# gillet-thomas/NeuroViT

Hardware: AMD Instinct MI355X
Metric: fMRI volumes/sec (fwd+bwd) ViT3D 128^3 p16 d768 L12 [timed step = fwd+bwd+AdamW update] (higher is better)
Workload: dtype bf16; 1 GPU; ViT3D-base 128^3 patch 16, train step (fwd+bwd+AdamW), batch 4/GPU, dropout 0; global_batch=4, parallelism=dp1, grad_buckets=7, grad_allreduce=none (1 GPU)

## Files before the change

### neurovit_amd/_cabi.py

```python
from __future__ import annotations

import ctypes
import os
import re
from typing import Dict, List, Tuple

_HERE = os.path.dirname(os.path.abspath(__file__))
HEADER = os.path.join(os.path.dirname(_HERE), "include", "neurovit_hip.h")
LIB_PATH = os.environ.get("NEUROVIT_HIP_LIB") or os.path.join(_HERE, "lib", "libneurovit_hip.so")

_SCALARS = {"int": ctypes.c_int, "long": ctypes.c_long, "float": ctypes.c_float, "double": ctypes.c_double}


class VitConfig(ctypes.Structure):
    _fields_ = [("image_size", ctypes.c_int), ("image_patch_size", ctypes.c_int), ("frames", ctypes.c_int),
                ("frame_patch_size", ctypes.c_int), ("channels", ctypes.c_int), ("num_classes", ctypes.c_int),
                ("dim", ctypes.c_int), ("depth", ctypes.c_int), ("heads", ctypes.c_int), ("dim_head", ctypes.c_int),
                ("mlp_dim", ctypes.c_int), ("ln_eps", ctypes.c_float), ("pool_mean", ctypes.c_int),
                ("image_width", ctypes.c_int), ("patch_width", ctypes.c_int),
                ("no_proj_dropout", ctypes.c_int)]


class VitInput(ctypes.Structure):
    _fields_ = [("vol_sigma", ctypes.c_void_p), ("time_points", ctypes.c_int), ("rows_form", ctypes.c_int), ("attn_export", ctypes.c_void_p)]
# ... 47 lines not shown
ABI_VERSION = 8


def parse_header(path: str = HEADER) -> Dict[str, Tuple[object, List[object]]]:
    src = open(path).read()
    src = re.sub(r"/\*.*?\*/", " ", src, flags=re.S)
    protos = {}
    for m in re.finditer(r"\b(int|long|const char\s*\*)\s+(nv_\w+)\s*\(([^;{]*?)\)\s*;", src, flags=re.S):
        ret, name, args = m.group(1), m.group(2), " ".join(m.group(3).split())
        restype = ctypes.c_char_p if "char" in ret else _SCALARS[ret]
        argtypes = []
        if args and args != "void":
            for a in args.split(","):
                a = a.strip()
                if "*" in a:
                    argtypes.append(ctypes.c_char_p if re.match(r"const char\s*\*", a) else ctypes.c_void_p)
                elif a.startswith("unsigned long"):
                    argtypes.append(ctypes.c_ulong)
                else:
                    argtypes.append(_SCALARS[a.split()[0]])
        protos[name] = (restype, argtypes)
    return protos


class _Lib:
    def __init__(self):
        self._dll = None
        self.protos = parse_header()

    def load(self):
        if self._dll is None:
            if not os.path.exists(LIB_PATH):
                raise RuntimeError(
                    f"neurovit_amd: {LIB_PATH} not found - build it with `python -c 'import __graft_entry__ as g; g.build()'` "
                    "(or `make -C neurovit_amd/csrc`). There is no CPU / PyTorch fallback for this path.")
            dll = ctypes.CDLL(LIB_PATH)
            for name, (restype, argtypes) in self.protos.items():
                fn = getattr(dll, name)
                fn.restype, fn.argtypes = restype, argtypes
            got = dll.nv_abi_version()
            if got != ABI_VERSION:
                raise RuntimeError(f"neurovit_amd: {LIB_PATH} has ABI revision {got}, this binding expects {ABI_VERSION} - rebuild the library "
                                   "(make -C neurovit_amd/csrc); see INTEGRATION.md 'ABI revisions'")
            if os.environ.get("NEUROVIT_ATTN_MODE"):
                dll.nv_attn_set_mode(int(os.environ["NEUROVIT_ATTN_MODE"]))
            if os.environ.get("NEUROVIT_ADAMW_WGS"):
                dll.nv_gemm_set_tile(12, int(os.environ["NEUROVIT_ADAMW_WGS"]))
            if os.environ.get("NEUROVIT_HEAD_STEP"):
                dll.nv_vit_set_head_step(int(os.environ["NEUROVIT_HEAD_STEP"]))
            if os.environ.get("NEUROVIT_WGRAD_WGS"):
                dll.nv_gemm_set_tile(14, int(os.environ["NEUROVIT_WGRAD_WGS"]))
            if os.environ.get("NEUROVIT_PATCH_MODE"):
                dll.nv_patch_set_mode(int(os.environ["NEUROVIT_PATCH_MODE"]))
            if os.environ.get("NEUROVIT_ADAMW_CAP"):
                dll.nv_gemm_set_tile(13, int(os.environ["NEUROVIT_ADAMW_CAP"]))
            self._dll = dll
        return self._dll

    def __getattr__(self, name):
        return getattr(self.load(), name)


lib = _Lib()


OPERAND_FORMATS = {"bf16": 0, "fp16": 1}
_operand_format = "bf16"


def set_operand_format(fmt: str) -> None:
    global _operand_format
    if fmt != _operand_format:
        if fmt not in OPERAND_FORMATS:
            raise ValueError(f"neurovit_amd: operand format must be 'bf16' or 'fp16', got {fmt!r}")
        check(lib.nv_set_operand_format(OPERAND_FORMATS[fmt]), "nv_set_operand_format")
        _operand_format = fmt


def operand_format() -> str:
    return _operand_format


def last_error() -> str:
    return (lib.nv_last_error() or b"").decode()


def check(rc: int, what: str = "") -> None:
    if rc != 0:
        raise RuntimeError(f"neurovit_amd C-ABI call failed ({what}, rc={rc}): {last_error()}")


def require_gpu() -> None:
    import torch
    if not torch.cuda.is_available():
        raise RuntimeError("neurovit_amd: no HIP device available - this path only runs on MI355X (gfx950); "
                           "there is no CPU fallback.")
    if lib.nv_arch_ok() != 1:
        raise RuntimeError(f"neurovit_amd: current device is not gfx950: {last_error()}")
```

### neurovit_amd/csrc/gemm.hip

```cpp
#include "gemm_common.h"
#include "gemm_pp.h"

template <typename T, int BM, int BN, bool A_T, bool B_T, int EPI>
__global__ __launch_bounds__(NTHREADS) void gemm_bf16_kernel(const GemmArgs g) {
  extern __shared__ __attribute__((aligned(16))) char smem[];
  constexpr int A_BYTES = BM * BK * 2, B_BYTES = BN * BK * 2;
  constexpr int TM = BM / 2, TN = BN / 2;
  constexpr int MI = TM / 16, NI = TN / 16;
  const int tid = threadIdx.x, lane = tid & 63, wid = tid >> 6;
  const int wm = wid >> 1, wn = wid & 1;
  const int tiles_n = (g.N + BN - 1) / BN, tiles_m = (g.M + BM - 1) / BM;
  const int bid = xcd_remap(blockIdx.x, gridDim.x);
  const int m0 = (g.col_order ? bid % tiles_m : bid / tiles_n) * BM, n0 = (g.col_order ? bid / tiles_m : bid % tiles_n) * BN;
  const int nk = (g.K + BK - 1) / BK;

  char* sA0 = smem;
  char* sB0 = smem + A_BYTES;
  char* sA1 = smem + A_BYTES + B_BYTES;
  char* sB1 = smem + 2 * A_BYTES + B_BYTES;

  f32x4 acc[MI][NI];
#pragma unroll
  for (int i = 0; i < MI; ++i)
#pragma unroll
// ... 25 lines not shown
    dma_issue<BN>(pb, stepB, sB0, uwid);
  } else {
    gload_tail(0);
    swrite(sA0, sB0);
  }
  __syncthreads();

  for (int kt = 0; kt < nk; ++kt) {
    const char* a = (kt & 1) ? sA1 : sA0;
    const char* b = (kt & 1) ? sB1 : sB0;
    char* na = (kt & 1) ? sA0 : sA1;
    char* nb = (kt & 1) ? sB0 : sB1;
    const bool next_dma = kt + 1 < nfull, next_tail = (kt + 1 < nk) && !next_dma;
    if (next_dma) {
      dma_issue<BM>(pa, stepA, na, uwid);
      dma_issue<BN>(pb, stepB, nb, uwid);
    } else if (next_tail) {
      gload_tail(kt + 1);
    }
#pragma unroll
    for (int ks = 0; ks < 2; ++ks) {
      r16x8 af[MI], bfr[NI];
#pragma unroll
      for (int i = 0; i < MI; ++i) af[i] = read_frag<A_T, BM>(a, wm * TM + 16 * i, ks, lane);
#pragma unroll
      for (int j = 0; j < NI; ++j) bfr[j] = read_frag<B_T, BN>(b, wn * TN + 16 * j, ks, lane);
#pragma unroll
      for (int i = 0; i < MI; ++i)
#pragma unroll
        for (int j = 0; j < NI; ++j)
          acc[i][j] = mfma16<T>(bfr[j], af[i], acc[i][j]);
    }
    if (next_tail) swrite(na, nb);
    __syncthreads();
  }

  epilogue<EPI, T, MI, NI>(acc, g, m0 + wm * TM, n0 + wn * TN, lane);
}

constexpr int WS_THREADS = 512;

template <bool T, int BX>
__device__ __forceinline__ void ws_offsets(long ld, int rc0, int lw, int lane, int (&voff)[BX / 32]) {
#pragma unroll
  for (int i = 0; i < BX / 32; ++i) {
    const int I = lw + 4 * i;
    if constexpr (!T) {
      const int row = I * 8 + (lane >> 3), ch = (lane & 7) ^ ((lane >> 3) & 7);
      voff[i] = (int)((((long)(rc0 + row)) * ld + (ch << 3)) * 2);
    } else if constexpr (BX == 128) {
      const int krow = I * 4 + (lane >> 4);
      const int ch = (lane & 15) ^ (((krow & 3) << 2) | ((krow >> 2) & 3));
      voff[i] = (int)(((long)krow * ld + rc0 + (ch << 3)) * 2);
    } else {
      const int krow = I * 8 + (lane >> 3);
      const int ch = (lane & 7) ^ ((((krow >> 1) & 1) | (((krow >> 3) & 1) << 1)) << 1);
      voff[i] = (int)(((long)krow * ld + rc0 + (ch << 3)) * 2);
    }
  }
}
template <int N>
__device__ __forceinline__ void ws_issue(__amdgpu_buffer_rsrc_t rsrc, const int* voff, int soff, char* img, int lw) {
#pragma unroll
  for (int i = 0; i < N; ++i)
    __builtin_amdgcn_raw_ptr_buffer_load_lds(rsrc, (lds_void_t*)(img + (lw + 4 * i) * 1024), 16, voff[i], soff, 0, 0);
}
#define WS_VM(n) asm volatile("s_waitcnt vmcnt(" #n ")" ::: "memory")
template <int PIECES>
__device__ __forceinline__ void ws_wait_tiles_in_flight(int tiles) {
  static_assert(PIECES == 4 || PIECES == 6 || PIECES == 8 || PIECES == 12 || PIECES == 16, "unsupported DMA piece count");
  if constexpr (PIECES == 16) {
    switch (tiles) { case 0: WS_VM(0); break; case 1: WS_VM(16); break; case 2: WS_VM(32); break; default: WS_VM(48); }
  } else if constexpr (PIECES == 12) {
    switch (tiles) { case 0: WS_VM(0); break; case 1: WS_VM(12); break; case 2: WS_VM(24); break; case 3: WS_VM(36); break; default: WS_VM(48); }
  } else if constexpr (PIECES == 8) {
    switch (tiles) { case 0: WS_VM(0); break; case 1: WS_VM(8); break; case 2: WS_VM(16); break; case 3: WS_VM(24); break; case 4: WS_VM(32); break; default: WS_VM(40); }
  } else if constexpr (PIECES == 6) {
    switch (tiles) { case 0: WS_VM(0); break; case 1: WS_VM(6); break; case 2: WS_VM(12); break; case 3: WS_VM(18); break; case 4: WS_VM(24); break; default: WS_VM(30); }
  } else {
    switch (tiles) { case 0: WS_VM(0); break; case 1: WS_VM(4); break; case 2: WS_VM(8); break; case 3: WS_VM(12); break; case 4: WS_VM(16); break; default: WS_VM(20); }
  }
}
#undef WS_VM

template <typename T, int BM, int BN, int S, int KS, bool A_T, bool B_T, int EPI>
__device__ __forceinline__ void gemm_ws_body(const GemmArgs& g, const int bid) {
  extern __shared__ __attribute__((aligned(16))) char smem[];
  constexpr int A_BYTES = BM * BK * 2, SUB = (BM + BN) * BK * 2, STAGE = KS * SUB;
  constexpr int TM = BM / 2, TN = BN / 2, MI = TM / 16, NI = TN / 16;
  constexpr int PIECES = KS * (BM / 32 + BN / 32);
  constexpr int D = S - 1;
  static_assert(S >= 3 && S <= 7 && (KS == 1 || KS == 2), "ring geometry");
  const int tid = threadIdx.x, lane = tid & 63;
  const int wid = __builtin_amdgcn_readfirstlane(tid >> 6);
  const int tiles_n = (g.N + BN - 1) / BN, tiles_m = (g.M + BM - 1) / BM;
  const int m0 = (g.col_order ? bid % tiles_m : bid / tiles_n) * BM, n0 = (g.col_order ? bid / tiles_m : bid % tiles_n) * BN;
  const int nk = ((g.K + BK - 1) / BK + KS - 1) / KS;

  if (wid >= 4) {
    const int lw = wid - 4;
    const unsigned bytesA = (unsigned)((((long)(A_T ? g.K : g.M) - 1) * g.lda + (A_T ? g.M : g.K)) * 2);
    const unsigned bytesB = (unsigned)((((long)(B_T ? g.K : g.N) - 1) * g.ldb + (B_T ? g.N : g.K)) * 2);
    const __amdgpu_buffer_rsrc_t rA = __builtin_amdgcn_make_buffer_rsrc((void*)g.A, 0, bytesA, 0x00020000);
    const __amdgpu_buffer_rsrc_t rB = __builtin_amdgcn_make_buffer_rsrc((void*)g.B, 0, bytesB, 0x00020000);
    int voA[BM / 32], voB[BN / 32];
    ws_offsets<A_T, BM>(g.lda, m0, lw, lane, voA);
    ws_offsets<B_T, BN>(g.ldb, n0, lw, lane, voB);
    const int stepA = (int)((A_T ? (long)BK * g.lda : BK) * 2), stepB = (int)((B_T ? (long)BK * g.ldb : BK) * 2);
    auto issue_stage = [&](int t, char* dst) {
#pragma unroll
      for (int u = 0; u < KS; ++u) {
        ws_issue<BM / 32>(rA, voA, (t * KS + u) * stepA, dst + u * SUB, lw);
        ws_issue<BN / 32>(rB, voB, (t * KS + u) * stepB, dst + u * SUB + A_BYTES, lw);
      }
    };
    const int pre = nk < D ? nk : D;
    for (int t = 0; t < pre; ++t) issue_stage(t, smem + t * STAGE);
    ws_wait_tiles_in_flight<PIECES>(pre - 1);
    __builtin_amdgcn_s_barrier();
    int fs = D % S;
    for (int kt = 0; kt + 1 < nk; ++kt) {
      if (kt + D < nk) issue_stage(kt + D, smem + fs * STAGE);
      const int last = (kt + D < nk) ? kt + D : nk - 1;
      ws_wait_tiles_in_flight<PIECES>(last - (kt + 1) > 0 ? last - (kt + 1) : 0);
      __builtin_amdgcn_s_barrier();
      fs = (fs + 1 == S) ? 0 : fs + 1;
    }
    EpiRegs<EPI, BM, BN, WS_THREADS> er;
    epilogue_lds_request<EPI, BM, BN, WS_THREADS>(er, g, m0, n0, tid);
    __builtin_amdgcn_s_barrier();
    __builtin_amdgcn_s_barrier();
    epilogue_lds_finish<EPI, T, BM, BN, WS_THREADS>(smem, g, m0, n0, tid, er, reinterpret_cast<const float*>(smem + S * STAGE));
    return;
  }

  const int wm = wid >> 1, wn = wid & 1;
  f32x4 acc[MI][NI];
#pragma unroll
  for (int i = 0; i < MI; ++i)
#pragma unroll
    for (int j = 0; j < NI; ++j) acc[i][j] = f32x4{0.f, 0.f, 0.f, 0.f};
  r16x8 fa0[MI], fb0[NI], fa1[MI], fb1[NI];
  int ci = 0;
  char* cur = smem;
  char* nxt = smem + STAGE;

#define WS_READ(FA, FB, BUF, HS)                                                                                   \
  _Pragma("unroll") for (int i = 0; i < MI; ++i) FA[i] = read_frag<A_T, BM>(BUF + ((HS) >> 1) * SUB, wm * TM + 16 * i, (HS) & 1, lane); \
  _Pragma("unroll") for (int j = 0; j < NI; ++j) FB[j] = read_frag<B_T, BN>(BUF + ((HS) >> 1) * SUB + A_BYTES, wn * TN + 16 * j, (HS) & 1, lane);
#define WS_MFMA(FA, FB)                                                       \
  _Pragma("unroll") for (int i = 0; i < MI; ++i)                             \
    _Pragma("unroll") for (int j = 0; j < NI; ++j)                           \
      acc[i][j] = mfma16<T>(FB[j], FA[i], acc[i][j]);
#define SB __builtin_amdgcn_sched_barrier(0);
#define WS_ADVANCE ci = (ci + 1 == S) ? 0 : ci + 1; cur = nxt; nxt = smem + ((ci + 1 == S) ? 0 : ci + 1) * STAGE;

  if constexpr (epi_is_fold<EPI>()) {
    ln_rows_to_lds(g, m0, BM, reinterpret_cast<float*>(smem + S * STAGE), tid, 256);
    ln_cols_to_lds<BM, BN>(g, n0, reinterpret_cast<float*>(smem + S * STAGE), 255 - tid);
    asm volatile("s_waitcnt lgkmcnt(0)" ::: "memory");
  }
  __builtin_amdgcn_s_barrier();
  if constexpr (KS == 1) {
    WS_READ(fa0, fb0, cur, 0)
    for (int kt = 0; kt + 1 < nk; ++kt) {
      WS_READ(fa1, fb1, cur, 1)
      SB WS_MFMA(fa0, fb0) SB
      asm volatile("s_waitcnt lgkmcnt(0)" ::: "memory");
      __builtin_amdgcn_s_barrier();
      SB WS_READ(fa0, fb0, nxt, 0)
      SB WS_MFMA(fa1, fb1) SB
      WS_ADVANCE
    }
    WS_READ(fa1, fb1, cur, 1)
    SB WS_MFMA(fa0, fb0) SB
    asm volatile("s_waitcnt lgkmcnt(0)" ::: "memory");
    __builtin_amdgcn_s_barrier();
    WS_MFMA(fa1, fb1)
  } else {
    r16x8 fa2[MI], fb2[NI];
#define WS_STAGE(A0, B0, A1, B1, A2, B2)                                      \
    WS_READ(A2, B2, cur, 2)                                                   \
    SB WS_MFMA(A0, B0) SB                                                     \
    WS_READ(A0, B0, cur, 3)                                                   \
    SB WS_MFMA(A1, B1) SB                                                     \
    WS_MFMA(A2, B2) SB                                                        \
    asm volatile("s_waitcnt lgkmcnt(0)" ::: "memory");                        \
    __builtin_amdgcn_s_barrier();                                             \
    SB WS_READ(A1, B1, nxt, 0)                                                \
    WS_READ(A2, B2, nxt, 1)                                                   \
    SB WS_MFMA(A0, B0) SB                                                     \
    WS_ADVANCE
    WS_READ(fa0, fb0, cur, 0)
    WS_READ(fa1, fb1, cur, 1)
    int kt = 0;
    for (; kt + 3 <= nk; kt += 3) {
      WS_STAGE(fa0, fb0, fa1, fb1, fa2, fb2)
      WS_STAGE(fa1, fb1, fa2, fb2, fa0, fb0)
      WS_STAGE(fa2, fb2, fa0, fb0, fa1, fb1)
    }
    if (kt + 1 <= nk) {
      WS_STAGE(fa0, fb0, fa1, fb1, fa2, fb2)
      if (kt + 2 <= nk) { WS_STAGE(fa1, fb1, fa2, fb2, fa0, fb0) }
    }
#undef WS_STAGE
    asm volatile("s_waitcnt lgkmcnt(0)" ::: "memory");
  }
#undef WS_READ
#undef WS_MFMA
#undef SB
#undef WS_ADVANCE
  static_assert(BM * cpitch<BN>() + colsum_scratch_bytes<BM, BN, WS_THREADS>() <= S * STAGE, "C tile (+ column-sum scratch) must fit in the ring");
  EpiRegs<EPI, BM, BN, WS_THREADS> er;
  epilogue_lds_request<EPI, BM, BN, WS_THREADS>(er, g, m0, n0, tid);
  park_acc<MI, NI, BN>(acc, smem, wm * TM, wn * TN, lane);
  asm volatile("s_waitcnt lgkmcnt(0)" ::: "memory");
  __builtin_amdgcn_s_barrier();
  epilogue_lds_finish<EPI, T, BM, BN, WS_THREADS>(smem, g, m0, n0, tid, er, reinterpret_cast<const float*>(smem + S * STAGE));
}

template <typename T, int BM, int BN, int S, int KS, bool A_T, bool B_T, int EPI>
__global__ __launch_bounds__(WS_THREADS) void gemm_ws_kernel(const GemmArgs g) {
  gemm_ws_body<T, BM, BN, S, KS, A_T, B_T, EPI>(g, xcd_remap(blockIdx.x, gridDim.x));
}

template <typename T, int BM, int BN, int S, int KS, bool A_T, bool B_T, int EPI>
__global__ __launch_bounds__(WS_THREADS) void gemm_ws_grouped_kernel(const GemmGroup G) {
  const int bid = xcd_remap(blockIdx.x, gridDim.x);
  int p = 0;
  while (p + 1 < G.count && bid >= G.tile_end[p]) ++p;
  gemm_ws_body<T, BM, BN, S, KS, A_T, B_T, EPI>(G.p[p], bid - (p ? G.tile_end[p - 1] : 0));
}

static int g_ring_override = 0;
static int g_tile_override = 0;
static int g_pp_grouped = 1;
static int g_pp_min_tiles = 128;
static int g_pq_min_tiles = 768;
extern "C" int nv_gemm_set_tile(int bm, int bn) {
  if (bm == 6) { g_pp_min_tiles = bn; return 0; }
  if (bm == 7) { g_pp_grouped = bn; return 0; }
  if (bm == 8) { g_pp_dbg = bn; return 0; }
  if (bm == 10) { g_pq_min_tiles = bn; return 0; }
  if (bm == 11) { g_pp_w32 = bn ? 1 : 0; return 0; }
  if (bm == 12) { g_pp_adamw_wgs = bn > 0 ? bn : 0; return 0; }
  if (bm == 14) { g_pp_wgrad_wgs = bn > 0 ? bn : 0; return 0; }
  if (bm == 13) { extern int g_adamw_ranges_cap; g_adamw_ranges_cap = bn > 0 ? bn : 0; return 0; }
  const bool small = (bm == 64 && (bn == 64 || bn == 128)) || (bm == 128 && bn == 128);
  NV_CHECK_ARG(bm == 0 || bm == 1 || (bm >= 3 && bm <= 5) || bm == 9 || small, "nv_gemm_set_tile: (%d, %d) is not a compiled tile", bm, bn);
  NV_CHECK_ARG(!(bm == 1 || bm == 3) || bn == 0 || bn == 1 || (bm == 3 && bn == 3), "nv_gemm_set_tile: ring %d is not compiled for tile %d", bn, bm);
  g_tile_override = (bm == 0) ? 0 : ((bm <= 5 || bm == 9) ? bm : bm * 1000 + bn);
  g_ring_override = (bm == 1 || bm == 3) ? bn : 0;
  return 0;
}

template <typename T, int BM, int BN, bool A_T, bool B_T, int EPI>
static int launch_tile(const GemmArgs& a, hipStream_t s) {
  constexpr int LDS = 2 * (BM + BN) * BK * 2;
  const int tiles = ((a.M + BM - 1) / BM) * ((a.N + BN - 1) / BN);
  auto kern = gemm_bf16_kernel<T, BM, BN, A_T, B_T, EPI>;
  static bool attr_set = false;
  if (!attr_set) {
    (void)hipFuncSetAttribute(reinterpret_cast<const void*>(kern), hipFuncAttributeMaxDynamicSharedMemorySize, LDS);
    attr_set = true;
  }
  const int slot = nv_prof_begin((A_T ? 2 : (B_T ? 1 : 0)), 2.0 * a.M * a.N * a.K, s);
  nv_prof_bytes(slot, gemm_algo_bytes(a, EPI, 2));
  hipLaunchKernelGGL(kern, dim3(tiles), dim3(NTHREADS), LDS, s, a);
  nv_prof_end(slot, s);
  NV_CHECK_LAUNCH("nv_gemm_bf16");
  return NV_OK;
}

template <typename T, int BM, int BN, int S, int KS, bool A_T, bool B_T, int EPI>
static int launch_ws(const GemmArgs& a, hipStream_t s) {
  constexpr int LDS = S * KS * (BM + BN) * BK * 2 + ln_rows_bytes<EPI, BM, BN>();
  static_assert(LDS <= 160 * 1024, "LDS ring too large");
  const int tiles = ((a.M + BM - 1) / BM) * ((a.N + BN - 1) / BN);
  auto kern = gemm_ws_kernel<T, BM, BN, S, KS, A_T, B_T, EPI>;
  static bool attr_set = false;
  if (!attr_set) {
    (void)hipFuncSetAttribute(reinterpret_cast<const void*>(kern), hipFuncAttributeMaxDynamicSharedMemorySize, LDS);
    attr_set = true;
  }
  const int slot = nv_prof_begin((A_T ? 2 : (B_T ? 1 : 0)), 2.0 * a.M * a.N * a.K, s);
  nv_prof_bytes(slot, gemm_algo_bytes(a, EPI, 2));
  hipLaunchKernelGGL(kern, dim3(tiles), dim3(WS_THREADS), LDS, s, a);
  nv_prof_end(slot, s);
  NV_CHECK_LAUNCH("nv_gemm_bf16/ws");
  return NV_OK;
}

struct GemmPlan { int family, ws, ring, sel, bm; };
static GemmPlan plan_gemm(bool A_T, bool B_T, int epi, int M, int N, int K, long lda, long ldb) {
  GemmPlan p{0, 0, 0, 0, 0};
  const bool k_ok = (K % BK == 0) || (A_T && B_T);
  const long rowsA = A_T ? K : M, rowsB = B_T ? K : N;
  const bool fits = rowsA * lda < (1L << 30) && rowsB * ldb < (1L << 30);
  const long t128 = (long)((M + 127) / 128) * ((N + 127) / 128);
  const long tpp = (long)((M + PP_BM - 1) / PP_BM) * ((N + PP_BN - 1) / PP_BN);
  const long tpq = (long)((M + PQ_BM - 1) / PQ_BM) * ((N + PQ_BN - 1) / PQ_BN);
  const bool pq_shape = !A_T && !B_T && (epi == EPI_STORE_BF16 || epi == EPI_STORE_F32 || epi == EPI_BIAS_F32);
  if (k_ok && fits && (g_tile_override == 9 || (g_tile_override == 0 && pq_shape && tpq >= g_pq_min_tiles))) {
    p.family = 3; p.bm = 128;
    return p;
  }
  if (k_ok && fits && (g_tile_override == 4 || (g_tile_override == 0 && tpp >= g_pp_min_tiles))) {
    p.family = 2; p.bm = PP_BM;
    return p;
  }
  if (k_ok && fits && g_tile_override < 1000) {
    int ws = (g_tile_override >= 4) ? 0 : g_tile_override;
    const long t64x128w = (long)((M + 63) / 64) * ((N + 127) / 128);
    if (ws == 0 && (t128 >= 32 || t64x128w >= 48)) ws = (t128 >= 1024) ? 1 : 3;
    int ring = g_ring_override;
    const bool k128_ok = ((K % (2 * BK)) == 0) || (A_T && B_T);
    const long t64x128 = (long)((M + 63) / 64) * ((N + 127) / 128);
    if (ring == 0) ring = (k128_ok && t64x128 <= 256 && K >= 1536) ? 3 : 1;
    if (ring == 3 && !k128_ok) ring = 1;
    if (ws >= 1 && ws <= 3) {
      p.family = 1; p.ws = ws; p.ring = ring; p.bm = (ws == 3) ? 64 : 128;
      return p;
    }
  }
  p.sel = g_tile_override >= 1000 ? g_tile_override : 0;
  if (!p.sel) {
    const long t64x128 = (long)((M + 63) / 64) * ((N + 127) / 128);
    p.sel = (t128 >= 1024) ? 128128 : (t64x128 >= 768 ? 64128 : 64064);
  }
  return p;
}

template <typename T, bool A_T, bool B_T, int EPI>
static int launch_fmt(const GemmArgs& a, hipStream_t s) {
  const GemmPlan p = plan_gemm(A_T, B_T, EPI, a.M, a.N, a.K, a.lda, a.ldb);
  if (p.family == 3) return launch_pq(A_T ? 2 : (B_T ? 1 : 0), EPI, a, s);
  if (p.family == 2) return launch_pp(A_T ? 2 : (B_T ? 1 : 0), EPI, a, s);
  if (p.family == 1) {
    const int ws = p.ws, ring = p.ring;
    if (ws == 1) return launch_ws<T, 128, 128, 3, 1, A_T, B_T, EPI>(a, s);
    return ring == 3 ? launch_ws<T, 64, 128, 3, 2, A_T, B_T, EPI>(a, s) : launch_ws<T, 64, 128, 3, 1, A_T, B_T, EPI>(a, s);
  }
  if constexpr (EPI == EPI_DGELU_COLSUM) {
    nv_set_error("nv_gemm_bf16: the fused column-sum epilogue needs a large-tile kernel for this shape (ask nv_gemm_tile_rows first)");
    return NV_ERR_ARG;
  } else {
    switch (p.sel) {
      case 128128: return launch_tile<T, 128, 128, A_T, B_T, EPI>(a, s);
      case 64128: return launch_tile<T, 64, 128, A_T, B_T, EPI>(a, s);
      default: return launch_tile<T, 64, 64, A_T, B_T, EPI>(a, s);
    }
  }
}

template <bool A_T, bool B_T, int EPI>
static int launch(const GemmArgs& a, hipStream_t s) {
  NV_DISPATCH_OPERAND(T, return launch_fmt<T, A_T, B_T, EPI>(a, s));
}

template <typename T, int EPI>
static int launch_fold_fmt(const GemmArgs& a, hipStream_t s) {
  const GemmPlan p = plan_gemm(false, false, EPI, a.M, a.N, a.K, a.lda, a.ldb);
  if (p.family == 2) return launch_pp(0, EPI, a, s);
  if (p.family == 1) {
    if (p.ws == 1) return launch_ws<T, 128, 128, 3, 1, false, false, EPI>(a, s);
    return p.ring == 3 ? launch_ws<T, 64, 128, 3, 2, false, false, EPI>(a, s) : launch_ws<T, 64, 128, 3, 1, false, false, EPI>(a, s);
  }
  nv_set_error("nv_gemm_lnfold: no LDS-epilogue kernel runs this shape (M=%d N=%d K=%d): ask nv_gemm_lnfold_supported first", a.M, a.N, a.K);
  return NV_ERR_ARG;
}
extern "C" int nv_gemm_lnfold_supported(int M, int N, int K) {
  if (M <= 0 || N <= 0 || K <= 0 || (N % 8) || (K % 8)) return 0;
  const GemmPlan p = plan_gemm(false, false, EPI_LNFOLD_STORE, M, N, K, K, K);
  return (p.family == 1 || p.family == 2) ? 1 : 0;
}
extern "C" long nv_ln_fold_stats_floats(int M, int d) { return 2L * M * ((d + 127) / 128); }

static void fold_args(GemmArgs& a, int M, int N, int K, const void* A, long lda, const void* W, long ldw, const float* bias) {
  a.A = (const r16*)A; a.B = (const r16*)W; a.bias = bias; a.aux_in = nullptr; a.aux_out = nullptr; a.aux_out2 = nullptr;
  a.lda = lda; a.ldb = ldw; a.ld_aux_in = 0; a.ld_aux_out = 0; a.ld_aux_out2 = 0;
  a.M = M; a.N = N; a.K = K; a.accumulate = 0; a.alpha = 1.f; a.drop = make_drop(0, 0.f); a.colscale = nullptr;
  a.col_order = (N > M) ? 1 : 0;
}

extern "C" int nv_gemm_resid_ln(int M, int N, int K, const void* A, long lda, const void* W, long ldw, const float* bias, const float* resid, long ldr, float* out,
                                long ldo, void* out16, long ldo16, float* stats, void* stream) {
  NV_CHECK_ARG(M > 0 && N > 0 && K > 0 && A && W && bias && resid && out && out16 && stats, "nv_gemm_resid_ln: null pointer / empty problem");
  NV_CHECK_ARG(nv_aligned16(A) && nv_aligned16(W) && nv_aligned16(bias) && nv_aligned16(resid) && nv_aligned16(out) && ((uintptr_t)out16 & 7) == 0 && nv_aligned16(stats) &&
                   (lda % 8) == 0 && (ldw % 8) == 0 && (ldr % 4) == 0 && (ldo % 4) == 0 && (ldo16 % 4) == 0 && (N % 8) == 0 && (K % 8) == 0 && lda >= K && ldw >= K && ldo >= N && ldo16 >= N,
               "nv_gemm_resid_ln: alignment / leading dimensions");
  GemmArgs a;
  fold_args(a, M, N, K, A, lda, W, ldw, bias);
// ... 201 lines not shown
```

### neurovit_amd/csrc/gemm_common.h

```cpp
#pragma once
#include "common.h"

enum {
  EPI_STORE_BF16 = 0,
  EPI_STORE_F32 = 1,
  EPI_BIAS_F32 = 2,
  EPI_BIAS_GELU = 3,
  EPI_BIAS_RESID = 4,
  EPI_DGELU = 5,
  EPI_BIAS_GELU_F8 = 7,
  EPI_BIAS_GELU_F8T = 8,
  EPI_DGELU_COLSUM = 6,
  EPI_BIAS_RESID_LN = 10,
  EPI_LNFOLD_STORE = 11,
  EPI_LNFOLD_GELU = 12,
  EPI_ADAMW = 9,
};

struct OptFuse {
  float* p = nullptr; float* m = nullptr; float* v = nullptr; r16* p16 = nullptr;
  AdamArgs a = {};
  int keep_grad = 0;
};

struct GemmArgs {
  const r16* A;
  const r16* B;
  void* C;
  const float* bias;
  const void* aux_in;
  void* aux_out;
  void* aux_out2;
  long lda, ldb, ldc, ld_aux_in, ld_aux_out, ld_aux_out2;
  int M, N, K;
  int accumulate;
  DropCfg drop;
  int col_order;
  float alpha;
  const float* colscale;
  OptFuse opt;
  const float* ln_stats = nullptr;
  const float* ln_cs = nullptr;
  int ln_tiles = 0;
  float ln_eps = 0.f;
};

static inline double gemm_algo_bytes(const GemmArgs& a, int epi, int operand_bytes) {
  const double mn = (double)a.M * a.N;
  double b = ((double)a.M * a.K + (double)a.N * a.K) * operand_bytes;
  switch (epi) {
    case EPI_STORE_BF16: b += mn * 2; break;
    case EPI_STORE_F32: b += mn * 4 * (a.accumulate ? 2 : 1) + (a.aux_out ? mn * 2 : 0); break;
    case EPI_BIAS_F32: b += mn * 4; break;
    case EPI_BIAS_GELU: b += mn * 2 + (a.aux_out ? mn * 2 : 0); break;
    case EPI_BIAS_RESID: b += mn * 8; break;
    case EPI_DGELU: case EPI_DGELU_COLSUM: b += mn * 4; break;
    case EPI_BIAS_GELU_F8: b += mn; break;
    case EPI_BIAS_GELU_F8T: b += mn * 5; break;
    case EPI_ADAMW: b += mn * (26 + (a.opt.keep_grad ? 4 : 0)); break;
    case EPI_BIAS_RESID_LN: b += mn * 10; break;
    case EPI_LNFOLD_STORE: case EPI_LNFOLD_GELU: b += mn * 2 + (double)a.M * a.ln_tiles * 8; break;
    default: break;
  }
  return b;
}

constexpr int BK = 64;
constexpr int NTHREADS = 256;
typedef __attribute__((address_space(3))) void lds_void_t;

__device__ __forceinline__ int img128t_off(int row, int chunk) {
  return row * 128 + ((chunk ^ ((((row >> 1) & 1) | (((row >> 3) & 1) << 1)) << 1)) << 4);
}

template <int BX>
__device__ __forceinline__ int imgT_off(int krow, int chunk) {
  if constexpr (BX == 128) return img256_off(krow, chunk);
  else return img128t_off(krow, chunk);
}

template <int BX, bool TAIL>
__device__ __forceinline__ void gload_rowmajor(const r16* X, long ld, int R, int K, int r0, int k0, int tid, uint4 (&reg)[BX / 32]) {
#pragma unroll
  for (int i = 0; i < BX / 32; ++i) {
    const int c = tid + NTHREADS * i;
    const int row = min(r0 + (c >> 3), R - 1), kk = k0 + ((c & 7) << 3);
    if constexpr (TAIL) {
      const bool ok = kk < K;
      const uint4 v = *reinterpret_cast<const uint4*>(X + (long)row * ld + (ok ? kk : 0));
      reg[i] = ok ? v : make_uint4(0, 0, 0, 0);
    } else {
      reg[i] = *reinterpret_cast<const uint4*>(X + (long)row * ld + kk);
    }
  }
}
template <int BX, bool TAIL>
__device__ __forceinline__ void gload_kmajor(const r16* X, long ld, int Ccols, int K, int c0, int k0, int tid, uint4 (&reg)[BX / 32]) {
  constexpr int CPR = BX / 8;
#pragma unroll
  for (int i = 0; i < BX / 32; ++i) {
    const int c = tid + NTHREADS * i;
    const int kk = k0 + c / CPR, col = min(c0 + ((c % CPR) << 3), Ccols - 8);
    if constexpr (TAIL) {
      const bool ok = kk < K;
      const uint4 v = *reinterpret_cast<const uint4*>(X + (long)(ok ? kk : 0) * ld + col);
      reg[i] = ok ? v : make_uint4(0, 0, 0, 0);
    } else {
      reg[i] = *reinterpret_cast<const uint4*>(X + (long)kk * ld + col);
    }
  }
}
template <int BX>
__device__ __forceinline__ void swrite_rowmajor(char* img, int tid, const uint4 (&reg)[BX / 32]) {
#pragma unroll
  for (int i = 0; i < BX / 32; ++i) {
    const int c = tid + NTHREADS * i;
    *reinterpret_cast<uint4*>(img + img128_off(c >> 3, c & 7)) = reg[i];
  }
}
template <int BX>
__device__ __forceinline__ void swrite_kmajor(char* img, int tid, const uint4 (&reg)[BX / 32]) {
  constexpr int CPR = BX / 8;
#pragma unroll
  for (int i = 0; i < BX / 32; ++i) {
    const int c = tid + NTHREADS * i;
    *reinterpret_cast<uint4*>(img + imgT_off<BX>(c / CPR, c % CPR)) = reg[i];
  }
}

typedef __attribute__((address_space(1))) const void gbl_void_t;
// ... 220 lines not shown
    n = tot;
  };
  if (g.ln_tiles <= LN_TILES_INFLIGHT) {
    f32x2 part[LN_TILES_INFLIGHT];
#pragma unroll
    for (int t = 0; t < LN_TILES_INFLIGHT; ++t)
      part[t] = (t < g.ln_tiles) ? *reinterpret_cast<const f32x2*>(g.ln_stats + ((long)t * g.M + m) * 2) : f32x2{0.f, 0.f};
#pragma unroll
    for (int t = 0; t < LN_TILES_INFLIGHT; ++t)
      if (t < g.ln_tiles) merge(t, part[t][0], part[t][1]);
  } else {
    for (int t = 0; t < g.ln_tiles; ++t) merge(t, g.ln_stats[((long)t * g.M + m) * 2], g.ln_stats[((long)t * g.M + m) * 2 + 1]);
  }
  mu = mean;
  rstd = 1.0f / sqrtf(m2 / (float)g.K + g.ln_eps);
}
__device__ __forceinline__ void ln_rows_to_lds(const GemmArgs& g, int m0, int BM, float* dst, int t, int nthreads) {
  for (int r = t; r < BM; r += nthreads) {
    float mu = 0.f, rstd = 0.f;
    if (m0 + r < g.M) ln_row_stats(g, m0 + r, mu, rstd);
    dst[2 * r] = mu; dst[2 * r + 1] = rstd;
  }
}
__device__ __forceinline__ float dpp_fold(float v, const int ctrl_sel) {
  int o;
  if (ctrl_sel == 0) o = __builtin_amdgcn_update_dpp(0, __builtin_bit_cast(int, v), 0xB1, 0xF, 0xF, true);
  else if (ctrl_sel == 1) o = __builtin_amdgcn_update_dpp(0, __builtin_bit_cast(int, v), 0x4E, 0xF, 0xF, true);
  else if (ctrl_sel == 2) o = __builtin_amdgcn_update_dpp(0, __builtin_bit_cast(int, v), 0x141, 0xF, 0xF, true);
  else o = __builtin_amdgcn_update_dpp(0, __builtin_bit_cast(int, v), 0x140, 0xF, 0xF, true);
  return v + __builtin_bit_cast(float, o);
}
__device__ __forceinline__ float half_wave_sum(float v) {
  v = dpp_fold(v, 0); v = dpp_fold(v, 1); v = dpp_fold(v, 2); v = dpp_fold(v, 3);
  float a = v, b = v;
  asm volatile("s_nop 1\n\tv_permlane16_swap_b32 %0, %1\n\ts_nop 0" : "+v"(a), "+v"(b));
  return a + b;
}

template <int EPI> constexpr bool epi_is_fold() { return EPI == EPI_LNFOLD_STORE || EPI == EPI_LNFOLD_GELU; }
template <int EPI, int BM, int BN = 128> constexpr int ln_rows_bytes() { return epi_is_fold<EPI>() ? BM * 8 + BN * 8 : 0; }
template <int BM, int BN>
__device__ __forceinline__ void ln_cols_to_lds(const GemmArgs& g, int n0, float* lnrow, int t) {
  if (t < BN / 2) {
    const int which = t / (BN / 4), n = n0 + (t % (BN / 4)) * 4;
    f32x4 v = f32x4{0.f, 0.f, 0.f, 0.f};
    if (n < g.N) v = *reinterpret_cast<const f32x4*>((which ? g.bias : g.ln_cs) + n);
    *reinterpret_cast<f32x4*>(lnrow + 2 * BM + which * BN + (t % (BN / 4)) * 4) = v;
  }
}

template <int EPI, int BM, int BN, int NT>
struct EpiRegs {
  static constexpr int CPR = BN / 4, RPS = NT / CPR, SLOTS = (BM + RPS - 1) / RPS;
  EpiCols cols;
  epi_aux_t<EPI> aux[SLOTS];
};
template <int EPI> constexpr bool epi_requests() { return !epi_is_fold<EPI>() && EPI != EPI_ADAMW; }

template <int EPI, int BM, int BN, int NT>
__device__ __forceinline__ void epilogue_lds_request(EpiRegs<EPI, BM, BN, NT>& er, const GemmArgs& g, int m0, int n0, int tid) {
  typedef EpiRegs<EPI, BM, BN, NT> R;
  static_assert(NT % R::CPR == 0 && 64 % R::CPR == 0, "every thread keeps one column group");
  if constexpr (epi_requests<EPI>()) {
    const int n = min(n0 + (tid % R::CPR) * 4, g.N - 4);
    er.cols = epi_load_cols<EPI>(g, n);
    if constexpr (epi_aux_kind<EPI>() != 0) {
      if (epi_aux_wanted<EPI>(g)) {
#pragma unroll
        for (int s = 0; s < R::SLOTS; ++s) er.aux[s] = epi_load_aux<EPI>(g, min(m0 + tid / R::CPR + s * R::RPS, g.M - 1), n);
      }
    }
  }
}

template <int EPI, typename T, int BM, int BN, int NT>
__device__ __forceinline__ void epilogue_lds_finish(char* ctile, const GemmArgs& g, int m0, int n0, int tid, const EpiRegs<EPI, BM, BN, NT>& er,
                                                    const float* lnrow = nullptr) {
  if constexpr (EPI == EPI_ADAMW) { epilogue_lds_adamw<T, BM, BN, NT>(ctile, g, m0, n0, tid); return; }
  typedef EpiRegs<EPI, BM, BN, NT> R;
  constexpr int CPR = R::CPR;
  constexpr bool FOLD = epi_is_fold<EPI>();
  float* scr = reinterpret_cast<float*>(ctile + BM * cpitch<BN>());
  f32x4 csum = f32x4{0.f, 0.f, 0.f, 0.f};
  static_assert(EPI != EPI_BIAS_RESID_LN || ((BM * CPR) % 64 == 0 && NT % 64 == 0 && CPR == 32 && BN == 128), "whole waves leave the loop together; 32 lanes share a row");
  const int col = (tid % CPR) * 4, n = n0 + col;
  if constexpr (epi_requests<EPI>()) __builtin_amdgcn_s_waitcnt(0x0F70);
#pragma unroll
  for (int s = 0; s < R::SLOTS; ++s) {
    const int row = tid / CPR + s * R::RPS;
    if (BM % R::RPS != 0 && row >= BM) break;
    const int m = m0 + row;
    f32x4 r = f32x4{0.f, 0.f, 0.f, 0.f};
    if (m < g.M && n < g.N) {
      const f32x4 cell = *reinterpret_cast<const f32x4*>(ctile + row * cpitch<BN>() + col * 4);
      if constexpr (FOLD) {
        const float mu = lnrow[2 * row], rstd = lnrow[2 * row + 1];
        const f32x4 y = (cell - mu * *reinterpret_cast<const f32x4*>(lnrow + 2 * BM + col)) * rstd + *reinterpret_cast<const f32x4*>(lnrow + 2 * BM + BN + col);
        if constexpr (EPI == EPI_LNFOLD_GELU) *reinterpret_cast<r16x4*>((r16*)g.C + (long)m * g.ldc + n) = cvt4<T>(gelu_f(y[0]), gelu_f(y[1]), gelu_f(y[2]), gelu_f(y[3]));
        else *reinterpret_cast<r16x4*>((r16*)g.C + (long)m * g.ldc + n) = cvt4<T>(y[0], y[1], y[2], y[3]);
      } else {
        r = epilogue4<EPI, T>(cell, g, m, n, er.cols, er.aux[s]);
        if constexpr (EPI == EPI_DGELU_COLSUM) csum += r;
      }
    }
    if constexpr (EPI == EPI_BIAS_RESID_LN) {
      float s1 = (r[0] + r[1]) + (r[2] + r[3]), s2 = __builtin_fmaf(r[0], r[0], r[1] * r[1]) + __builtin_fmaf(r[2], r[2], r[3] * r[3]);
      s1 = half_wave_sum(s1); s2 = half_wave_sum(s2);
      if ((tid & 31) == 0 && m < g.M) {
        float* out = (float*)g.aux_out2 + ((long)(n0 / BN) * g.M + m) * 2;
        out[0] = s1; out[1] = s2;
      }
    }
  }
  if constexpr (EPI == EPI_DGELU_COLSUM) {
#pragma unroll
    for (int o = 32; o >= CPR; o >>= 1) {
      csum[0] += __shfl_xor(csum[0], o, 64); csum[1] += __shfl_xor(csum[1], o, 64);
      csum[2] += __shfl_xor(csum[2], o, 64); csum[3] += __shfl_xor(csum[3], o, 64);
    }
    const int lane = tid & 63, wave = tid >> 6;
    if (lane < CPR) *reinterpret_cast<f32x4*>(scr + wave * BN + lane * 4) = csum;
    __syncthreads();
    if (tid < BN && n0 + tid < g.N && m0 < g.M) {
      float s = 0.f;
#pragma unroll
      for (int w = 0; w < NT / 64; ++w) s += scr[w * BN + tid];
      ((float*)g.aux_out)[(long)(m0 / BM) * g.ld_aux_out + n0 + tid] = s;
    }
  }
}

template <int EPI, typename T, int BM, int BN, int NT>
__device__ __forceinline__ void epilogue_lds(char* ctile, const GemmArgs& g, int m0, int n0, int tid, const float* lnrow = nullptr) {
  EpiRegs<EPI, BM, BN, NT> er;
  epilogue_lds_request<EPI, BM, BN, NT>(er, g, m0, n0, tid);
  epilogue_lds_finish<EPI, T, BM, BN, NT>(ctile, g, m0, n0, tid, er, lnrow);
}


// ... 7 lines not shown
```

Before: 1190 volumes/s.

## Add 64x96 warp-specialized GEMM tile with carried remainder rows for small grids

Adds a 64x96 GEMM tile variant for the BIAS_RESID and STORE_F32 epilogues. It carries a 16-row remainder block into the last M tile, so M values just above a multiple of 64 (e.g. 257 tokens per volume times batch) do not launch a mostly empty extra tile row. A heuristic picks this tile when the baseline plan would be the 64x128 ring-3 tile with K>=1536 and the tile count fits within one wave of CUs, with the aim of filling the GPU better. In exchange it needs new LDS swizzle offsets, a 10-piece DMA wait count, and an epilogue where some threads sit idle, all of which are extra code paths that could be subtly wrong.

```diff
diff --git a/neurovit_amd/_cabi.py b/neurovit_amd/_cabi.py
--- a/neurovit_amd/_cabi.py
+++ b/neurovit_amd/_cabi.py
@@ -123,6 +123,8 @@
                 dll.nv_gemm_set_tile(14, int(os.environ["NEUROVIT_WGRAD_WGS"]))
             if os.environ.get("NEUROVIT_PATCH_MODE"):
                 dll.nv_patch_set_mode(int(os.environ["NEUROVIT_PATCH_MODE"]))
+            if os.environ.get("NEUROVIT_TILE96"):
+                dll.nv_gemm_set_tile(15, int(os.environ["NEUROVIT_TILE96"]))
             if os.environ.get("NEUROVIT_ADAMW_CAP"):
                 dll.nv_gemm_set_tile(13, int(os.environ["NEUROVIT_ADAMW_CAP"]))
             self._dll = dll
diff --git a/neurovit_amd/csrc/gemm.hip b/neurovit_amd/csrc/gemm.hip
--- a/neurovit_amd/csrc/gemm.hip
+++ b/neurovit_amd/csrc/gemm.hip
@@ -101,6 +101,10 @@
       const int krow = I * 4 + (lane >> 4);
       const int ch = (lane & 15) ^ (((krow & 3) << 2) | ((krow >> 2) & 3));
       voff[i] = (int)(((long)krow * ld + rc0 + (ch << 3)) * 2);
+    } else if constexpr (BX == 96) {
+      const int pos = I * 64 + lane, krow = pos / 12;
+      const int ch = (pos - krow * 12) ^ (((krow >> 3) & 1) << 1);
+      voff[i] = (int)(((long)krow * ld + rc0 + (ch << 3)) * 2);
     } else {
       const int krow = I * 8 + (lane >> 3);
       const int ch = (lane & 7) ^ ((((krow >> 1) & 1) | (((krow >> 3) & 1) << 1)) << 1);
@@ -117,8 +121,10 @@
 #define WS_VM(n) asm volatile("s_waitcnt vmcnt(" #n ")" ::: "memory")
 template <int PIECES>
 __device__ __forceinline__ void ws_wait_tiles_in_flight(int tiles) {
-  static_assert(PIECES == 4 || PIECES == 6 || PIECES == 8 || PIECES == 12 || PIECES == 16, "unsupported DMA piece count");
-  if constexpr (PIECES == 16) {
+  static_assert(PIECES == 4 || PIECES == 6 || PIECES == 8 || PIECES == 10 || PIECES == 12 || PIECES == 16, "unsupported DMA piece count");
+  if constexpr (PIECES == 10) {
+    switch (tiles) { case 0: WS_VM(0); break; case 1: WS_VM(10); break; case 2: WS_VM(20); break; case 3: WS_VM(30); break; default: WS_VM(40); }
+  } else if constexpr (PIECES == 16) {
     switch (tiles) { case 0: WS_VM(0); break; case 1: WS_VM(16); break; case 2: WS_VM(32); break; default: WS_VM(48); }
   } else if constexpr (PIECES == 12) {
     switch (tiles) { case 0: WS_VM(0); break; case 1: WS_VM(12); break; case 2: WS_VM(24); break; case 3: WS_VM(36); break; default: WS_VM(48); }
@@ -132,17 +138,19 @@
 }
 #undef WS_VM
 
-template <typename T, int BM, int BN, int S, int KS, bool A_T, bool B_T, int EPI>
-__device__ __forceinline__ void gemm_ws_body(const GemmArgs& g, const int bid) {
+template <typename T, int BM, int BN, int S, int KS, bool A_T, bool B_T, int EPI, int XR = 0, int MI_ = BM / 32>
+__device__ __forceinline__ void gemm_ws_body(const GemmArgs& g, const int bid, const int tile_rows = 0) {
   extern __shared__ __attribute__((aligned(16))) char smem[];
-  constexpr int A_BYTES = BM * BK * 2, SUB = (BM + BN) * BK * 2, STAGE = KS * SUB;
-  constexpr int TM = BM / 2, TN = BN / 2, MI = TM / 16, NI = TN / 16;
-  constexpr int PIECES = KS * (BM / 32 + BN / 32);
+  constexpr int AR = XR ? BM + 32 : BM, RM = BM + XR;
+  constexpr int A_BYTES = AR * BK * 2, SUB = (AR + BN) * BK * 2, STAGE = KS * SUB;
+  constexpr int TM = BM / 2, TN = BN / 2, MI = MI_, NI = TN / 16;
+  constexpr int PIECES = KS * (AR / 32 + BN / 32);
   constexpr int D = S - 1;
   static_assert(S >= 3 && S <= 7 && (KS == 1 || KS == 2), "ring geometry");
+  static_assert(XR == 0 || (XR == 16 && !A_T && !epi_is_fold<EPI>()), "carried rows: one 16-row block of a row-major A");
   const int tid = threadIdx.x, lane = tid & 63;
   const int wid = __builtin_amdgcn_readfirstlane(tid >> 6);
-  const int tiles_n = (g.N + BN - 1) / BN, tiles_m = (g.M + BM - 1) / BM;
+  const int tiles_n = (g.N + BN - 1) / BN, tiles_m = tile_rows ? tile_rows : (g.M + BM - 1) / BM;
   const int m0 = (g.col_order ? bid % tiles_m : bid / tiles_n) * BM, n0 = (g.col_order ? bid / tiles_m : bid % tiles_n) * BN;
   const int nk = ((g.K + BK - 1) / BK + KS - 1) / KS;
 
@@ -152,14 +160,14 @@
     const unsigned bytesB = (unsigned)((((long)(B_T ? g.K : g.N) - 1) * g.ldb + (B_T ? g.N : g.K)) * 2);
     const __amdgpu_buffer_rsrc_t rA = __builtin_amdgcn_make_buffer_rsrc((void*)g.A, 0, bytesA, 0x00020000);
     const __amdgpu_buffer_rsrc_t rB = __builtin_amdgcn_make_buffer_rsrc((void*)g.B, 0, bytesB, 0x00020000);
-    int voA[BM / 32], voB[BN / 32];
-    ws_offsets<A_T, BM>(g.lda, m0, lw, lane, voA);
+    int voA[AR / 32], voB[BN / 32];
+    ws_offsets<A_T, AR>(g.lda, m0, lw, lane, voA);
     ws_offsets<B_T, BN>(g.ldb, n0, lw, lane, voB);
     const int stepA = (int)((A_T ? (long)BK * g.lda : BK) * 2), stepB = (int)((B_T ? (long)BK * g.ldb : BK) * 2);
     auto issue_stage = [&](int t, char* dst) {
 #pragma unroll
       for (int u = 0; u < KS; ++u) {
-        ws_issue<BM / 32>(rA, voA, (t * KS + u) * stepA, dst + u * SUB, lw);
+        ws_issue<AR / 32>(rA, voA, (t * KS + u) * stepA, dst + u * SUB, lw);
         ws_issue<BN / 32>(rB, voB, (t * KS + u) * stepB, dst + u * SUB + A_BYTES, lw);
       }
     };
@@ -175,11 +183,11 @@
       __builtin_amdgcn_s_barrier();
       fs = (fs + 1 == S) ? 0 : fs + 1;
     }
-    EpiRegs<EPI, BM, BN, WS_THREADS> er;
-    epilogue_lds_request<EPI, BM, BN, WS_THREADS>(er, g, m0, n0, tid);
+    EpiRegs<EPI, RM, BN, WS_THREADS> er;
+    epilogue_lds_request<EPI, RM, BN, WS_THREADS>(er, g, m0, n0, tid);
     __builtin_amdgcn_s_barrier();
     __builtin_amdgcn_s_barrier();
-    epilogue_lds_finish<EPI, T, BM, BN, WS_THREADS>(smem, g, m0, n0, tid, er, reinterpret_cast<const float*>(smem + S * STAGE));
+    epilogue_lds_finish<EPI, T, RM, BN, WS_THREADS>(smem, g, m0, n0, tid, er, reinterpret_cast<const float*>(smem + S * STAGE));
     return;
   }
 
@@ -195,7 +203,7 @@
   char* nxt = smem + STAGE;
 
 #define WS_READ(FA, FB, BUF, HS)                                                                                   \
-  _Pragma("unroll") for (int i = 0; i < MI; ++i) FA[i] = read_frag<A_T, BM>(BUF + ((HS) >> 1) * SUB, wm * TM + 16 * i, (HS) & 1, lane); \
+  _Pragma("unroll") for (int i = 0; i < MI; ++i) FA[i] = read_frag<A_T, AR>(BUF + ((HS) >> 1) * SUB, wm * TM + 16 * i, (HS) & 1, lane); \
   _Pragma("unroll") for (int j = 0; j < NI; ++j) FB[j] = read_frag<B_T, BN>(BUF + ((HS) >> 1) * SUB + A_BYTES, wn * TN + 16 * j, (HS) & 1, lane);
 #define WS_MFMA(FA, FB)                                                       \
   _Pragma("unroll") for (int i = 0; i < MI; ++i)                             \
@@ -259,13 +267,31 @@
 #undef WS_MFMA
 #undef SB
 #undef WS_ADVANCE
-  static_assert(BM * cpitch<BN>() + colsum_scratch_bytes<BM, BN, WS_THREADS>() <= S * STAGE, "C tile (+ column-sum scratch) must fit in the ring");
-  EpiRegs<EPI, BM, BN, WS_THREADS> er;
-  epilogue_lds_request<EPI, BM, BN, WS_THREADS>(er, g, m0, n0, tid);
+  static_assert(RM * cpitch<BN>() + colsum_scratch_bytes<RM, BN, WS_THREADS>() <= S * STAGE, "C tile (+ column-sum scratch) must fit in the ring");
+  EpiRegs<EPI, RM, BN, WS_THREADS> er;
+  epilogue_lds_request<EPI, RM, BN, WS_THREADS>(er, g, m0, n0, tid);
   park_acc<MI, NI, BN>(acc, smem, wm * TM, wn * TN, lane);
   asm volatile("s_waitcnt lgkmcnt(0)" ::: "memory");
   __builtin_amdgcn_s_barrier();
-  epilogue_lds_finish<EPI, T, BM, BN, WS_THREADS>(smem, g, m0, n0, tid, er, reinterpret_cast<const float*>(smem + S * STAGE));
+  epilogue_lds_finish<EPI, T, RM, BN, WS_THREADS>(smem, g, m0, n0, tid, er, reinterpret_cast<const float*>(smem + S * STAGE));
+}
+
+__host__ __device__ inline bool ws96_carries(int M) { return M >= 64 && (M % 64) >= 1 && (M % 64) <= 16; }
+__host__ __device__ inline int ws96_tiles_m(int M) { return ws96_carries(M) ? M / 64 : (M + 63) / 64; }
+
+template <typename T, bool B_T, int EPI>
+__global__ __launch_bounds__(WS_THREADS) void gemm_ws96_kernel(const GemmArgs g) {
+  constexpr int BM = 64, BN = 96;
+  const int bid = xcd_remap(blockIdx.x, gridDim.x);
+  const int tiles_m = ws96_tiles_m(g.M), tiles_n = (g.N + BN - 1) / BN;
+  const int tm = g.col_order ? bid % tiles_m : bid / tiles_n;
+  if (tm == tiles_m - 1 && ws96_carries(g.M)) {
+    const int wid = __builtin_amdgcn_readfirstlane(threadIdx.x >> 6);
+    if (wid == 2 || wid == 3) gemm_ws_body<T, BM, BN, 3, 2, false, B_T, EPI, 16, 3>(g, bid, tiles_m);
+    else gemm_ws_body<T, BM, BN, 3, 2, false, B_T, EPI, 16, 2>(g, bid, tiles_m);
+  } else {
+    gemm_ws_body<T, BM, BN, 3, 2, false, B_T, EPI, 0>(g, bid, tiles_m);
+  }
 }
 
 template <typename T, int BM, int BN, int S, int KS, bool A_T, bool B_T, int EPI>
@@ -283,6 +309,8 @@
 
 static int g_ring_override = 0;
 static int g_tile_override = 0;
+static int g_tile96 = 1;
+static int g_tile96_launches = 0;
 static int g_pp_grouped = 1;
 static int g_pp_min_tiles = 128;
 static int g_pq_min_tiles = 768;
@@ -294,6 +322,12 @@
   if (bm == 11) { g_pp_w32 = bn ? 1 : 0; return 0; }
   if (bm == 12) { g_pp_adamw_wgs = bn > 0 ? bn : 0; return 0; }
   if (bm == 14) { g_pp_wgrad_wgs = bn > 0 ? bn : 0; return 0; }
+  if (bm == 15) {
+    NV_CHECK_ARG(bn >= 0 && bn <= 2, "nv_gemm_set_tile: (15, %d): 0 heuristic, 1 never, 2 always", bn);
+    g_tile96 = bn;
+    return 0;
+  }
+  if (bm == 16) return g_tile96_launches;
   if (bm == 13) { extern int g_adamw_ranges_cap; g_adamw_ranges_cap = bn > 0 ? bn : 0; return 0; }
   const bool small = (bm == 64 && (bn == 64 || bn == 128)) || (bm == 128 && bn == 128);
   NV_CHECK_ARG(bm == 0 || bm == 1 || (bm >= 3 && bm <= 5) || bm == 9 || small, "nv_gemm_set_tile: (%d, %d) is not a compiled tile", bm, bn);
@@ -340,6 +374,37 @@
   return NV_OK;
 }
 
+template <typename T, bool B_T, int EPI>
+static int launch_ws96(const GemmArgs& a, hipStream_t s) {
+  constexpr int BM = 64, BN = 96;
+  constexpr int LDS = 3 * 2 * (BM + BN) * BK * 2, LDS_CARRY = 3 * 2 * (BM + 32 + BN) * BK * 2;
+  static_assert(LDS_CARRY <= 160 * 1024, "LDS ring too large");
+  const int tiles = ws96_tiles_m(a.M) * ((a.N + BN - 1) / BN);
+  auto kern = gemm_ws96_kernel<T, B_T, EPI>;
+  static bool attr_set = false;
+  if (!attr_set) {
+    (void)hipFuncSetAttribute(reinterpret_cast<const void*>(kern), hipFuncAttributeMaxDynamicSharedMemorySize, LDS_CARRY);
+    attr_set = true;
+  }
+  const int slot = nv_prof_begin(B_T ? 1 : 0, 2.0 * a.M * a.N * a.K, s);
+  nv_prof_bytes(slot, gemm_algo_bytes(a, EPI, 2));
+  hipLaunchKernelGGL(kern, dim3(tiles), dim3(WS_THREADS), ws96_carries(a.M) ? LDS_CARRY : LDS, s, a);
+  nv_prof_end(slot, s);
+  NV_CHECK_LAUNCH("nv_gemm_bf16/ws96");
+  ++g_tile96_launches;
+  return NV_OK;
+}
+
+static int device_cu_count() {
+  static int n = -1;
+  if (n < 0) {
+    int dev = 0, v = 0;
+    if (hipGetDevice(&dev) == hipSuccess && hipDeviceGetAttribute(&v, hipDeviceAttributeMultiprocessorCount, dev) == hipSuccess) n = v;
+    else { (void)hipGetLastError(); return 0; }
+  }
+  return n;
+}
+
 struct GemmPlan { int family, ws, ring, sel, bm; };
 static GemmPlan plan_gemm(bool A_T, bool B_T, int epi, int M, int N, int K, long lda, long ldb) {
   GemmPlan p{0, 0, 0, 0, 0};
@@ -349,6 +414,12 @@
   const long t128 = (long)((M + 127) / 128) * ((N + 127) / 128);
   const long tpp = (long)((M + PP_BM - 1) / PP_BM) * ((N + PP_BN - 1) / PP_BN);
   const long tpq = (long)((M + PQ_BM - 1) / PQ_BM) * ((N + PQ_BN - 1) / PQ_BN);
+  const bool k128_ok = ((K % (2 * BK)) == 0) || (A_T && B_T);
+  const bool t96_ok = k_ok && fits && k128_ok && !A_T && (N % 96) == 0 && ((!B_T && epi == EPI_BIAS_RESID) || (B_T && epi == EPI_STORE_F32));
+  if (t96_ok && g_tile96 == 2) {
+    p.family = 1; p.ws = 4; p.ring = 3; p.bm = 64;
+    return p;
+  }
   const bool pq_shape = !A_T && !B_T && (epi == EPI_STORE_BF16 || epi == EPI_STORE_F32 || epi == EPI_BIAS_F32);
   if (k_ok && fits && (g_tile_override == 9 || (g_tile_override == 0 && pq_shape && tpq >= g_pq_min_tiles))) {
     p.family = 3; p.bm = 128;
@@ -363,10 +434,14 @@
     const long t64x128w = (long)((M + 63) / 64) * ((N + 127) / 128);
     if (ws == 0 && (t128 >= 32 || t64x128w >= 48)) ws = (t128 >= 1024) ? 1 : 3;
     int ring = g_ring_override;
-    const bool k128_ok = ((K % (2 * BK)) == 0) || (A_T && B_T);
     const long t64x128 = (long)((M + 63) / 64) * ((N + 127) / 128);
     if (ring == 0) ring = (k128_ok && t64x128 <= 256 && K >= 1536) ? 3 : 1;
     if (ring == 3 && !k128_ok) ring = 1;
+    if (t96_ok && g_tile96 == 0 && g_tile_override == 0 && g_ring_override == 0 && ws == 3 && ring == 3 && K >= 1536 &&
+        (long)ws96_tiles_m(M) * (N / 96) <= device_cu_count()) {
+      p.family = 1; p.ws = 4; p.ring = 3; p.bm = 64;
+      return p;
+    }
     if (ws >= 1 && ws <= 3) {
       p.family = 1; p.ws = ws; p.ring = ring; p.bm = (ws == 3) ? 64 : 128;
       return p;
@@ -387,6 +462,9 @@
   if (p.family == 2) return launch_pp(A_T ? 2 : (B_T ? 1 : 0), EPI, a, s);
   if (p.family == 1) {
     const int ws = p.ws, ring = p.ring;
+    if constexpr (!A_T && ((!B_T && EPI == EPI_BIAS_RESID) || (B_T && EPI == EPI_STORE_F32))) {
+      if (ws == 4) return launch_ws96<T, B_T, EPI>(a, s);
+    }
     if (ws == 1) return launch_ws<T, 128, 128, 3, 1, A_T, B_T, EPI>(a, s);
     return ring == 3 ? launch_ws<T, 64, 128, 3, 2, A_T, B_T, EPI>(a, s) : launch_ws<T, 64, 128, 3, 1, A_T, B_T, EPI>(a, s);
   }
diff --git a/neurovit_amd/csrc/gemm_common.h b/neurovit_amd/csrc/gemm_common.h
--- a/neurovit_amd/csrc/gemm_common.h
+++ b/neurovit_amd/csrc/gemm_common.h
@@ -73,9 +73,14 @@
   return row * 128 + ((chunk ^ ((((row >> 1) & 1) | (((row >> 3) & 1) << 1)) << 1)) << 4);
 }
 
+__device__ __forceinline__ int img192t_off(int row, int chunk) {
+  return row * 192 + ((chunk ^ (((row >> 3) & 1) << 1)) << 4);
+}
+
 template <int BX>
 __device__ __forceinline__ int imgT_off(int krow, int chunk) {
   if constexpr (BX == 128) return img256_off(krow, chunk);
+  else if constexpr (BX == 96) return img192t_off(krow, chunk);
   else return img128t_off(krow, chunk);
 }
 
@@ -402,6 +407,7 @@
 template <int EPI, int BM, int BN, int NT>
 struct EpiRegs {
   static constexpr int CPR = BN / 4, RPS = NT / CPR, SLOTS = (BM + RPS - 1) / RPS;
+  static constexpr int ACTIVE = RPS * CPR;
   EpiCols cols;
   epi_aux_t<EPI> aux[SLOTS];
 };
@@ -410,7 +416,8 @@
 template <int EPI, int BM, int BN, int NT>
 __device__ __forceinline__ void epilogue_lds_request(EpiRegs<EPI, BM, BN, NT>& er, const GemmArgs& g, int m0, int n0, int tid) {
   typedef EpiRegs<EPI, BM, BN, NT> R;
-  static_assert(NT % R::CPR == 0 && 64 % R::CPR == 0, "every thread keeps one column group");
+  static_assert((NT % R::CPR == 0 && 64 % R::CPR == 0) || EPI == EPI_STORE_F32 || EPI == EPI_BIAS_RESID,
+                "every thread keeps one column group; only the per-element epilogues may leave threads out");
   if constexpr (epi_requests<EPI>()) {
     const int n = min(n0 + (tid % R::CPR) * 4, g.N - 4);
     er.cols = epi_load_cols<EPI>(g, n);
@@ -435,6 +442,9 @@
   static_assert(EPI != EPI_BIAS_RESID_LN || ((BM * CPR) % 64 == 0 && NT % 64 == 0 && CPR == 32 && BN == 128), "whole waves leave the loop together; 32 lanes share a row");
   const int col = (tid % CPR) * 4, n = n0 + col;
   if constexpr (epi_requests<EPI>()) __builtin_amdgcn_s_waitcnt(0x0F70);
+  if constexpr (R::ACTIVE != NT) {
+    if (tid >= R::ACTIVE) return;
+  }
 #pragma unroll
   for (int s = 0; s < R::SLOTS; ++s) {
     const int row = tid / CPR + s * R::RPS;
```

Result: no change. 1190 volumes/s (-0.1%).
